# XiSHEN0220/RANSAC-Flow

Measured on AMD Instinct MI355X. Metric: aligned image-pairs/sec @480×640, 1/2/4/8 MI355X; max-abs flow Δ vs ref, higher is better.
Workload: dtype f32

## Files before the change

include/rfx_api.h:

```cpp
#ifndef RFX_API_H
#define RFX_API_H

#include <stddef.h>
#include <stdint.h>

#ifdef __cplusplus
extern "C" {
#endif

#define RFX_OK 0
#define RFX_E_ARG (-1)
#define RFX_E_LIMIT (-2)

#define RFX_ACT_NONE 0
#define RFX_ACT_RELU 1
#define RFX_ACT_SIGMOID 2

const char* rfx_version(void);

#define RFX_ABI_VERSION 17
int rfx_abi_version(void);

int rfx_group_begin(void);
int rfx_group_end(void* stream);
int rfx_group_abort(void);
int rfx_group_side_streams(int enable);
int rfx_group_stats(long long* groups, long long* launches);

int rfx_conv2d_f32(const float* in, const float* wT, const int32_t* ktab, const float* scale,
                   const float* shift, const float* residual, float* out, int N, int Cin, int Hin,
                   int Win, int Cout, int KH, int KW, int stride, int pad, int act, void* stream);

int rfx_conv2d_tile_variant(int N, int Cout, int Hout, int Wout);

int rfx_conv2d_kernel_id(int N, int Cin, int Cout, int KH, int KW, int stride, int pad, int Hout, int Wout);

int rfx_conv3x3_f32(const float* in, const float* wP, const float* scale, const float* shift, const float* residual,
                    float* out, int N, int Cin, int H, int W, int Cout, int act, int k_chunk, void* stream);
int rfx_conv3x3_kernel_id(int N, int Cin, int Cout, int H, int W, int k_chunk);
int rfx_conv3x3_s2_f32(const float* in, const float* wP, const float* scale, const float* shift, const float* residual,
                       float* out, int N, int Cin, int H, int W, int Cout, int act, void* stream);

int rfx_conv3x3_conv1x1_kernel_id(int N, int H, int W, int Cmid);
int rfx_conv3x3_conv1x1_f32(const float* in, const float* wP2, const float* scale2, const float* shift2, int act2,
                            const float* wQ3, const float* scale3, const float* shift3, const float* residual, int act3,
                            float* out, int N, int Cin, int H, int W, int Cmid, int Cexp, void* stream);

int rfx_maxpool2d_f32(const float* in, float* out, int NC, int Hin, int Win, int k, int stride,
                      int pad, void* stream);

int rfx_blurpool2d_f32(const float* in, float* out, int NC, int Hin, int Win, int stride, void* stream);

int rfx_maxblurpool2d_f32(const float* in, float* out, int NC, int Hin, int Win, int stride, void* stream);

int rfx_stem_conv3x3_maxblur_f32(const float* in, const float* wT, const float* scale, const float* shift, float* out,
                                 int N, int H, int W, int Cout, void* stream);

int rfx_stem_conv7x7_maxpool_f32(const float* in, const float* wT, const float* scale, const float* shift, float* out,
                                 int N, int H, int W, int Cout, void* stream);

int rfx_l2norm_nchw_f32(const float* in, float* out, int N, int C, int HW, long long out_batch_stride,
                        long long out_chan_stride, void* stream);
int rfx_l2norm_nchw_scatter_f32(const float* in, float* out, int N, int C, int HW, const long long* dst_off,
                                long long out_chan_stride, void* stream);

int rfx_flow_head_f32(const float* logits, float* flow, int N, int K, int rows, int cols, void* stream);

int rfx_resize_bilinear_f32(const float* in, float* out, int NC, int Hin, int Win, int Hout, int Wout,
                            int align_corners, void* stream);

int rfx_lanczos_pass_u8(const uint8_t* in, uint8_t* out, int N, int inH, int inW, int outH, int outW, int C,
                        const int32_t* bounds, const int32_t* weights, int ksize, int vertical, int row_offset,
                        void* stream);

int rfx_u8_to_f32_chw(const uint8_t* in, float* raw, float* norm, int N, int H, int W, const float* mean3_host,
                      const float* std3_host, void* stream);

int rfx_copy_cols_f32(const float* src, float* dst, long long rows, int w_src, int w_dst, void* stream);

int rfx_corr_neigh_f32(const float* x, const float* y, float* out, int N, int C, int H, int W, int K,
                       void* stream);
int rfx_corr_neigh_variant_f32(const float* x, const float* y, float* out, int N, int C, int H, int W, int K,
                               int variant, void* stream);

int rfx_corr_neigh_bidir_f32(const float* x, const float* y, float* out_xy, float* out_yx, int N, int C, int H, int W, int K,
                             void* stream);
int rfx_corr_timing(int enable);
int rfx_corr_timing_collect(float* us_out, int cap);

int rfx_warp_grid_f32(const float* Hm, float* grid, int B, int h, int w, void* stream);

int rfx_grid_sample_f32(const float* in, const float* grid, float* out, int N, int C, int Hi, int Wi,
                        int Ho, int Wo, int align_corners, void* stream);

int rfx_compose_flow_f32(const float* flowDown, const float* coarseGrid, float* flow12, float* inb,
                         float* flowUp, int N, int hd, int wd, int Hc, int Wc, int H, int W, int clamp, void* stream);

int rfx_flow_grad_clamp_f32(const float* flowCoarse, const float* grid, float* flowGrad, float* flow, int B, int H, int W,
                            int grid_batch, void* stream);

int rfx_merge_multi_h_f32(const float* flow, const float* match12, long long match12_stride, const float* cyc,
                          const float* inb, int n, long long HW, float th, int multiH, float* flowGlobal,
                          float* matchGlobal, uint8_t* binary, void* stream);

int rfx_match_score_f32(const float* match12, long long match12_stride, const float* cyc, const float* inb, int n,
                        long long HW, float* score, void* stream);

size_t rfx_remove_small_cc_ws_bytes(int N, int H, int W);
int rfx_remove_small_cc_f32(const float* in, float* out, int N, int H, int W, float match_th, int max_area, void* ws,
                            void* stream);

size_t rfx_remove_small_cc_ragged_ws_bytes(long long total_px);
int rfx_remove_small_cc_ragged_f32(const float* in, float* out, const long long* match_off, const int32_t* dims, int n_active,
                                   long long total_px, long long max_hw, float match_th, void* ws, void* stream);

size_t rfx_nearest_fill_ws_bytes(int N, int H, int W);
int rfx_nearest_fill_f32(const float* values, const unsigned char* explained, float* out, int32_t* index, int N, int H, int W, int C,
                         void* ws, void* stream);

size_t rfx_flow_points_ws_bytes(int N, int H, int W);
int rfx_flow_points_f32(const float* flow, const unsigned char* keep, const unsigned char* bg, int N, int H, int W, int k, int wA,
                        int hA, int wB, int hB, float* pts1, long long* pts2, long long* offsets, void* ws, void* stream);
// ... 131 lines not shown
```

ransac-flow_amd/csrc/pool.hip:

```cpp
#include "common.h"
#include "group.h"
#include <math.h>

static inline int grid_for(long long total, int block) {
    long long g = (total + block - 1) / block;
    const long long cap = 256LL * 32;
    return (int)(g < cap ? g : cap);
}

__global__ __launch_bounds__(256) void maxpool2d_kernel(const float* __restrict__ in, float* __restrict__ out,
                                                        long long total, int Hin, int Win, int Hout, int Wout,
                                                        int k, int stride, int pad) {
    for (long long idx = (long long)blockIdx.x * blockDim.x + threadIdx.x; idx < total;
         idx += (long long)gridDim.x * blockDim.x) {
        const int ow = (int)(idx % Wout);
        const long long r = idx / Wout;
        const int oh = (int)(r % Hout);
        const long long nc = r / Hout;
        const float* src = in + nc * Hin * Win;
        float m = -INFINITY;
        const int ih0 = oh * stride - pad, iw0 = ow * stride - pad;
        for (int i = 0; i < k; ++i) {
            const int ih = ih0 + i;
            if ((unsigned)ih >= (unsigned)Hin) continue;
            for (int j = 0; j < k; ++j) {
                const int iw = iw0 + j;
                if ((unsigned)iw >= (unsigned)Win) continue;
                const float v = src[(size_t)ih * Win + iw];
                m = (v > m || v != v) ? v : m;
            }
        }
        out[idx] = m;
    }
}

extern "C" int rfx_maxpool2d_f32(const float* in, float* out, int NC, int Hin, int Win, int k, int stride,
                                 int pad, void* stream) {
    if (!in || !out || NC <= 0 || Hin <= 0 || Win <= 0 || k <= 0 || stride <= 0 || pad < 0 || pad > k / 2)
        return RFX_E_ARG;
    const int Hout = (Hin + 2 * pad - k) / stride + 1, Wout = (Win + 2 * pad - k) / stride + 1;
    if (Hout <= 0 || Wout <= 0) return RFX_E_ARG;
    const long long total = (long long)NC * Hout * Wout;
    hipLaunchKernelGGL(maxpool2d_kernel, dim3(grid_for(total, 256)), dim3(256), 0, rfx_stream(stream), in, out,
                       total, Hin, Win, Hout, Wout, k, stride, pad);
    RFX_LAUNCH_CHECK();
    return RFX_OK;
}

__device__ __forceinline__ int reflect1(int i, int n) {
    return i < 0 ? -i : (i >= n ? 2 * n - 2 - i : i);
}

struct PlaneArgs { const float* in; float* out; long long total; int Hin, Win, Hout, Wout, stride; };
struct L2NormArgs { const float* in; float* out; long long NP; int C, HW; long long obs, ocs; };
struct FlowHeadArgs { const float* logits; float* flow; long long NP; int K, rows, cols; };
struct ResizeArgs { const float* in; float* out; long long total; int Hin, Win, Hout, Wout; float sh, sw; int align; };

__device__ __forceinline__ void blurpool2d_body(const PlaneArgs& a, const unsigned bx, const unsigned gx) {
    const long long total = a.total;
    const int Hin = a.Hin, Win = a.Win, Hout = a.Hout, Wout = a.Wout, stride = a.stride;
    const float w[3] = {0.25f, 0.5f, 0.25f};
    [&](const float* __restrict__ in, float* __restrict__ out) {
    for (long long idx = (long long)bx * blockDim.x + threadIdx.x; idx < total;
         idx += (long long)gx * blockDim.x) {
        const int ow = (int)(idx % Wout);
        const long long r = idx / Wout;
        const int oh = (int)(r % Hout);
        const long long nc = r / Hout;
        const float* src = in + nc * Hin * Win;
        float acc = 0.0f;
#pragma unroll
        for (int i = 0; i < 3; ++i) {
            const int ih = reflect1(oh * stride - 1 + i, Hin);
#pragma unroll
            for (int j = 0; j < 3; ++j) {
                const int iw = reflect1(ow * stride - 1 + j, Win);
                acc = fmaf(src[(size_t)ih * Win + iw], w[i] * w[j], acc);
            }
        }
        out[idx] = acc;
    }
    }(a.in, a.out);
}

using BlurPool = RfxFamily<PlaneArgs, blurpool2d_body, 256>;
__global__ __launch_bounds__(BlurPool::BLOCK) void blurpool2d_kernel(PlaneArgs a) { blurpool2d_body(a, blockIdx.x, gridDim.x); }

extern "C" int rfx_blurpool2d_f32(const float* in, float* out, int NC, int Hin, int Win, int stride, void* stream) {
    if (!in || !out || NC <= 0 || Hin < 2 || Win < 2 || stride <= 0) return RFX_E_ARG;
    const int Hout = (Hin + 2 - 3) / stride + 1, Wout = (Win + 2 - 3) / stride + 1;
    const long long total = (long long)NC * Hout * Wout;
    const PlaneArgs a = {in, out, total, Hin, Win, Hout, Wout, stride};
    return BlurPool::launch(blurpool2d_kernel, a, (unsigned)grid_for(total, BlurPool::BLOCK), rfx_stream(stream));
}

__global__ __launch_bounds__(256) void maxblurpool2d_kernel(const float* __restrict__ in, float* __restrict__ out,
                                                            long long total, int Hin, int Win, int Hout, int Wout,
                                                            int stride) {
    const float w[3] = {0.25f, 0.5f, 0.25f};
    const int Hm = Hin - 1, Wm = Win - 1;
    for (long long idx = (long long)blockIdx.x * blockDim.x + threadIdx.x; idx < total;
         idx += (long long)gridDim.x * blockDim.x) {
        const int ow = (int)(idx % Wout);
        const long long r = idx / Wout;
        const int oh = (int)(r % Hout);
        const long long nc = r / Hout;
        const float* src = in + nc * Hin * Win;
        float acc = 0.0f;
#pragma unroll
        for (int i = 0; i < 3; ++i) {
            const int my = reflect1(oh * stride - 1 + i, Hm);
#pragma unroll
            for (int j = 0; j < 3; ++j) {
                const int mx = reflect1(ow * stride - 1 + j, Wm);
                const float* q = src + (size_t)my * Win + mx;
                const float a = q[0], b = q[1], c = q[Win], d = q[Win + 1];
                float m = a;
                m = (b > m || b != b) ? b : m;
                m = (c > m || c != c) ? c : m;
                m = (d > m || d != d) ? d : m;
                acc = fmaf(m, w[i] * w[j], acc);
            }
        }
        out[idx] = acc;
    }
}

__device__ __forceinline__ float maxblur_one(const float* __restrict__ src, int oh, int ow, int Win, int Hm, int Wm) {
    const float w[3] = {0.25f, 0.5f, 0.25f};
    float acc = 0.0f;
#pragma unroll
    for (int i = 0; i < 3; ++i) {
        const int my = reflect1(oh * 2 - 1 + i, Hm);
#pragma unroll
        for (int j = 0; j < 3; ++j) {
            const int mx = reflect1(ow * 2 - 1 + j, Wm);
            const float* q = src + (size_t)my * Win + mx;
            const float a = q[0], b = q[1], c = q[Win], d = q[Win + 1];
            float m = a;
            m = (b > m || b != b) ? b : m;
            m = (c > m || c != c) ? c : m;
            m = (d > m || d != d) ? d : m;
            acc = fmaf(m, w[i] * w[j], acc);
        }
    }
    return acc;
}

__global__ __launch_bounds__(256) void maxblurpool2d_s2_block_kernel(const float* __restrict__ in,
                                                                     float* __restrict__ out, long long nblocks,
                                                                     int Hin, int Win, int Hout, int Wout) {
    const float w[3] = {0.25f, 0.5f, 0.25f};
    const int Hm = Hin - 1, Wm = Win - 1;
    const int BH = (Hout + 1) / 2, BW = (Wout + 1) / 2;
    for (long long idx = (long long)blockIdx.x * blockDim.x + threadIdx.x; idx < nblocks;
         idx += (long long)gridDim.x * blockDim.x) {
        const int bx = (int)(idx % BW);
        const long long r = idx / BW;
        const int by = (int)(r % BH);
        const long long nc = r / BH;
        const float* src = in + nc * Hin * Win;
        float* dst = out + nc * Hout * Wout;
        const bool interior = by >= 1 && 4 * by + 4 <= Hin - 1 && bx >= 1 && 4 * bx + 8 <= Win && 2 * by + 1 < Hout &&
                              2 * bx + 1 < Wout;
        if (!interior) {
#pragma unroll
            for (int dy = 0; dy < 2; ++dy)
#pragma unroll
                for (int dx = 0; dx < 2; ++dx) {
                    const int oh = 2 * by + dy, ow = 2 * bx + dx;
                    if (oh < Hout && ow < Wout) dst[(size_t)oh * Wout + ow] = maxblur_one(src, oh, ow, Win, Hm, Wm);
                }
            continue;
        }
// ... 329 lines not shown
```

ransac-flow_amd/csrc/preproc.hip:

```cpp
#include "common.h"

namespace {

constexpr int PRECISION_BITS = 32 - 8 - 2;

__device__ __forceinline__ uint8_t clip8(int v) {
    v >>= PRECISION_BITS;
    return (uint8_t)(v < 0 ? 0 : (v > 255 ? 255 : v));
}

template <int CT>
__global__ __launch_bounds__(256) void lanczos_pass_kernel(const uint8_t* __restrict__ in, uint8_t* __restrict__ out,
                                                           long long total, int inH, int inW, int oH, int oW, int Crt,
                                                           const int32_t* __restrict__ bounds,
                                                           const int32_t* __restrict__ kk, int ksize, int vertical,
                                                           int row_off) {
    for (long long idx = (long long)blockIdx.x * blockDim.x + threadIdx.x; idx < total;
         idx += (long long)gridDim.x * blockDim.x) {
        const int ox = (int)(idx % oW);
        const long long r = idx / oW;
        const int oy = (int)(r % oH);
        const long long n = r / oH;
        const int C = CT ? CT : Crt;
        const uint8_t* src = in + (size_t)n * inH * inW * C;
        const int o = vertical ? oy : ox;
        const int lo = bounds[2 * o], cnt = bounds[2 * o + 1];
        const int32_t* k = kk + (size_t)o * ksize;
        int acc[4] = {1 << (PRECISION_BITS - 1), 1 << (PRECISION_BITS - 1), 1 << (PRECISION_BITS - 1),
                      1 << (PRECISION_BITS - 1)};
        if (vertical) {
            for (int j = 0; j < cnt; ++j) {
                const uint8_t* p = src + ((size_t)(lo + j) * inW + ox) * C;
                const int w = k[j];
#pragma unroll
                for (int c = 0; c < 4; ++c) if (c < C) acc[c] += (int)p[c] * w;
            }
        } else {
            const uint8_t* row = src + (size_t)(oy + row_off) * inW * C;
            for (int j = 0; j < cnt; ++j) {
                const uint8_t* p = row + (size_t)(lo + j) * C;
                const int w = k[j];
#pragma unroll
                for (int c = 0; c < 4; ++c) if (c < C) acc[c] += (int)p[c] * w;
            }
        }
        uint8_t* dst = out + (size_t)idx * C;
#pragma unroll
        for (int c = 0; c < 4; ++c) if (c < C) dst[c] = clip8(acc[c]);
    }
}

__global__ __launch_bounds__(256) void u8_to_f32_kernel(const uint8_t* __restrict__ in, float* __restrict__ raw,
                                                        float* __restrict__ norm, long long total, int HW, float m0,
                                                        float m1, float m2, float s0, float s1, float s2) {
    const float mean[3] = {m0, m1, m2}, sd[3] = {s0, s1, s2};
    for (long long idx = (long long)blockIdx.x * blockDim.x + threadIdx.x; idx < total;
         idx += (long long)gridDim.x * blockDim.x) {
        const long long n = idx / HW;
        const int px = (int)(idx - n * HW);
        const uint8_t* p = in + (size_t)idx * 3;
#pragma unroll
        for (int c = 0; c < 3; ++c) {
            const float v = __fdiv_rn((float)p[c], 255.0f);
            const size_t o = ((size_t)n * 3 + c) * HW + px;
            if (raw) raw[o] = v;
            if (norm) norm[o] = __fdiv_rn(__fsub_rn(v, mean[c]), sd[c]);
        }
    }
}

inline int grid_for(long long total) {
    long long g = (total + 255) / 256;
    return (int)(g < 8192 ? g : 8192);
}

}

extern "C" int rfx_lanczos_pass_u8(const uint8_t* in, uint8_t* out, int N, int inH, int inW, int outH, int outW, int C,
                                   const int32_t* bounds, const int32_t* weights, int ksize, int vertical, int row_offset,
                                   void* stream) {
    if (!in || !out || !bounds || !weights) return RFX_E_ARG;
    if (N <= 0 || inH <= 0 || inW <= 0 || outH <= 0 || outW <= 0 || C <= 0 || C > 4 || ksize <= 0 || row_offset < 0)
        return RFX_E_ARG;
    if (vertical ? (outW != inW) : (outH + row_offset > inH)) return RFX_E_ARG;
    const long long total = (long long)N * outH * outW;
    if (C == 3)
        hipLaunchKernelGGL(lanczos_pass_kernel<3>, dim3(grid_for(total)), dim3(256), 0, rfx_stream(stream), in, out, total, inH,
                           inW, outH, outW, C, bounds, weights, ksize, vertical, row_offset);
    else
        hipLaunchKernelGGL(lanczos_pass_kernel<0>, dim3(grid_for(total)), dim3(256), 0, rfx_stream(stream), in, out, total, inH,
                           inW, outH, outW, C, bounds, weights, ksize, vertical, row_offset);
    RFX_LAUNCH_CHECK();
    return RFX_OK;
}

extern "C" int rfx_u8_to_f32_chw(const uint8_t* in, float* raw, float* norm, int N, int H, int W, const float* mean3_host,
                                 const float* std3_host, void* stream) {
    if (!in || (!raw && !norm) || N <= 0 || H <= 0 || W <= 0) return RFX_E_ARG;
    if (norm && (!mean3_host || !std3_host)) return RFX_E_ARG;
    const float one[3] = {1.f, 1.f, 1.f}, zero[3] = {0.f, 0.f, 0.f};
    const float* m = mean3_host ? mean3_host : zero;
    const float* s = std3_host ? std3_host : one;
    const long long total = (long long)N * H * W;
    hipLaunchKernelGGL(u8_to_f32_kernel, dim3(grid_for(total)), dim3(256), 0, rfx_stream(stream), in, raw, norm, total,
                       H * W, m[0], m[1], m[2], s[0], s[1], s[2]);
    RFX_LAUNCH_CHECK();
    return RFX_OK;
}
```

ransac-flow_amd/rfx/_lib.py:

```python
import ctypes
import os
from ctypes import c_int, c_int32, c_int64, c_uint64, c_float, c_double, c_void_p, c_size_t, c_longlong, c_char_p

_HERE = os.path.dirname(os.path.abspath(__file__))
LIB_PATH = os.environ.get("RFX_LIB") or os.path.normpath(os.path.join(_HERE, "..", "librfx.so"))

SIGNATURES = {
    "rfx_version": (c_char_p, []),
    "rfx_abi_version": (c_int, []),
    "rfx_group_begin": (c_int, []),
    "rfx_group_end": (c_int, [c_void_p]),
    "rfx_group_abort": (c_int, []),
    "rfx_group_side_streams": (c_int, [c_int]),
    "rfx_group_stats": (c_int, [c_void_p, c_void_p]),
    "rfx_conv2d_f32": (c_int, [c_void_p] * 7 + [c_int] * 10 + [c_void_p]),
    "rfx_conv2d_dilated_f32": (c_int, [c_void_p] * 7 + [c_int] * 11 + [c_void_p]),
    "rfx_conv1x1_split_f32": (c_int, [c_void_p] * 6 + [c_int] * 5 + [c_void_p]),
    "rfx_conv3x3_split_f32": (c_int, [c_void_p] * 6 + [c_int] * 6 + [c_void_p]),
    "rfx_conv3x3_split_s2_f32": (c_int, [c_void_p] * 6 + [c_int] * 6 + [c_void_p]),
    "rfx_conv1x1_split_strided_f32": (c_int, [c_void_p] * 6 + [c_int] * 7 + [c_void_p]),
    "rfx_conv1x1_split_tile_channels": (c_int, [c_int] * 4),
    "rfx_conv1x1_expand64_f32": (c_int, [c_void_p] * 6 + [c_int] * 6 + [c_void_p]),
    "rfx_conv1x1_expand64_dual_f32": (c_int, [c_void_p] * 9 + [c_int] * 5 + [c_void_p]),
    "rfx_adaptive_avgpool2d_f32": (c_int, [c_void_p, c_void_p] + [c_int] * 5 + [c_void_p]),
    "rfx_softmax_accum_f32": (c_int, [c_void_p, c_void_p, c_int, c_int, c_longlong, c_float, c_int, c_void_p]),
    "rfx_argmax_mask_f32": (c_int, [c_void_p, c_int, c_int, c_longlong, c_int, c_int, c_void_p, c_void_p, c_void_p]),
    "rfx_conv2d_tile_variant": (c_int, [c_int] * 4),
    "rfx_conv2d_kernel_id": (c_int, [c_int] * 9),
    "rfx_conv3x3_f32": (c_int, [c_void_p] * 6 + [c_int] * 7 + [c_void_p]),
    "rfx_conv3x3_kernel_id": (c_int, [c_int] * 6),
    "rfx_conv3x3_s2_f32": (c_int, [c_void_p] * 6 + [c_int] * 6 + [c_void_p]),
    "rfx_conv3x3_conv1x1_kernel_id": (c_int, [c_int] * 4),
    "rfx_conv3x3_conv1x1_f32": (c_int, [c_void_p] * 4 + [c_int] + [c_void_p] * 4 + [c_int, c_void_p] + [c_int] * 6 + [c_void_p]),
    "rfx_maxpool2d_f32": (c_int, [c_void_p, c_void_p] + [c_int] * 6 + [c_void_p]),
    "rfx_blurpool2d_f32": (c_int, [c_void_p, c_void_p] + [c_int] * 4 + [c_void_p]),
    "rfx_maxblurpool2d_f32": (c_int, [c_void_p, c_void_p] + [c_int] * 4 + [c_void_p]),
    "rfx_stem_conv3x3_maxblur_f32": (c_int, [c_void_p] * 5 + [c_int] * 4 + [c_void_p]),
    "rfx_stem_conv7x7_maxpool_f32": (c_int, [c_void_p] * 5 + [c_int] * 4 + [c_void_p]),
    "rfx_l2norm_nchw_f32": (c_int, [c_void_p, c_void_p, c_int, c_int, c_int, c_longlong, c_longlong, c_void_p]),
    "rfx_l2norm_nchw_scatter_f32": (c_int, [c_void_p, c_void_p, c_int, c_int, c_int, c_void_p, c_longlong, c_void_p]),
    "rfx_flow_head_f32": (c_int, [c_void_p, c_void_p] + [c_int] * 4 + [c_void_p]),
    "rfx_resize_bilinear_f32": (c_int, [c_void_p, c_void_p] + [c_int] * 6 + [c_void_p]),
    "rfx_lanczos_pass_u8": (c_int, [c_void_p, c_void_p] + [c_int] * 6 + [c_void_p, c_void_p] + [c_int] * 3 + [c_void_p]),
    "rfx_u8_to_f32_chw": (c_int, [c_void_p] * 3 + [c_int] * 3 + [c_void_p] * 3),
    "rfx_copy_cols_f32": (c_int, [c_void_p, c_void_p, c_longlong, c_int, c_int, c_void_p]),
    "rfx_corr_neigh_f32": (c_int, [c_void_p] * 3 + [c_int] * 5 + [c_void_p]),
    "rfx_corr_neigh_variant_f32": (c_int, [c_void_p] * 3 + [c_int] * 6 + [c_void_p]),
    "rfx_corr_neigh_bidir_f32": (c_int, [c_void_p] * 4 + [c_int] * 5 + [c_void_p]),
    "rfx_corr_timing": (c_int, [c_int]),
    "rfx_corr_timing_collect": (c_int, [c_void_p, c_int]),
    "rfx_warp_grid_f32": (c_int, [c_void_p, c_void_p] + [c_int] * 3 + [c_void_p]),
    "rfx_grid_sample_f32": (c_int, [c_void_p] * 3 + [c_int] * 7 + [c_void_p]),
    "rfx_compose_flow_f32": (c_int, [c_void_p] * 5 + [c_int] * 8 + [c_void_p]),
    "rfx_flow_grad_clamp_f32": (c_int, [c_void_p] * 4 + [c_int] * 4 + [c_void_p]),
    "rfx_merge_multi_h_f32": (c_int, [c_void_p, c_void_p, c_longlong, c_void_p, c_void_p, c_int, c_longlong, c_float, c_int,
                                      c_void_p, c_void_p, c_void_p, c_void_p]),
    "rfx_match_score_f32": (c_int, [c_void_p, c_longlong, c_void_p, c_void_p, c_int, c_longlong, c_void_p, c_void_p]),
    "rfx_remove_small_cc_ws_bytes": (c_size_t, [c_int] * 3),
    "rfx_remove_small_cc_f32": (c_int, [c_void_p, c_void_p, c_int, c_int, c_int, c_float, c_int, c_void_p, c_void_p]),
    "rfx_remove_small_cc_ragged_ws_bytes": (c_size_t, [c_longlong]),
    "rfx_remove_small_cc_ragged_f32": (c_int, [c_void_p] * 4 + [c_int, c_longlong, c_longlong, c_float, c_void_p, c_void_p]),
    "rfx_nearest_fill_ws_bytes": (c_size_t, [c_int] * 3),
    "rfx_nearest_fill_f32": (c_int, [c_void_p] * 4 + [c_int] * 4 + [c_void_p, c_void_p]),
    "rfx_flow_points_ws_bytes": (c_size_t, [c_int] * 3),
    "rfx_flow_points_f32": (c_int, [c_void_p] * 3 + [c_int] * 8 + [c_void_p] * 5),
    "rfx_sample_points_f32": (c_int, [c_void_p] * 4 + [c_int] * 5 + [c_void_p] * 4),
    "rfx_epe_ws_bytes": (c_size_t, [c_int] * 3),
    "rfx_epe_homography_f32": (c_int, [c_void_p] * 2 + [c_int] * 3 + [c_void_p] * 5),
    "rfx_epe_flow_f32": (c_int, [c_void_p] * 4 + [c_int] * 3 + [c_void_p] * 5),
    "rfx_mutual_nn_ws_bytes": (c_size_t, [c_int, c_int]),
    "rfx_mutual_nn_f32": (c_int, [c_void_p, c_int, c_int, c_void_p, c_int, c_int, c_int] + [c_void_p] * 5 + [c_int, c_void_p]),
    "rfx_mutual_nn_batched_f32": (c_int, [c_void_p, c_int, c_int, c_longlong, c_void_p, c_int, c_int, c_longlong, c_int]
                                  + [c_void_p] * 5 + [c_int, c_int, c_void_p]),
    "rfx_mutual_nn_ragged_f32": (c_int, [c_void_p, c_int, c_void_p, c_int, c_void_p, c_void_p, c_int, c_int, c_int, c_void_p,
                                         c_void_p, c_void_p, c_int, c_void_p, c_void_p, c_int, c_int, c_void_p]),
    "rfx_dlt4_homography": (c_int, [c_void_p, c_void_p, c_int, c_void_p, c_void_p]),
    "rfx_prediction_f32": (c_int, [c_void_p, c_void_p, c_int, c_void_p, c_int, c_void_p, c_void_p]),
    "rfx_score_hypotheses": (c_int, [c_void_p, c_void_p, c_int, c_void_p, c_int, c_float] + [c_void_p] * 5),
    "rfx_ransac_ws_bytes": (c_size_t, [c_int, c_int]),
    "rfx_ransac_h4": (c_int, [c_void_p, c_void_p, c_int, c_void_p, c_int, c_float] + [c_void_p] * 5),
    "rfx_ransac_batched_ws_bytes": (c_size_t, [c_int, c_int, c_int]),
    "rfx_ransac_h4_batched_stage": (c_int, [c_void_p, c_void_p, c_void_p, c_int, c_void_p, c_int, c_float] + [c_void_p] * 4
                                    + [c_int, c_int, c_void_p]),
    "rfx_ransac_degenerate_gather": (c_int, [c_void_p] * 4 + [c_int, c_void_p, c_int, c_int] + [c_void_p] * 5 + [c_int, c_void_p]),
    "rfx_ransac_patch_h_rows": (c_int, [c_void_p, c_int, c_int, c_int] + [c_void_p] * 4 + [c_int, c_void_p]),
    "rfx_dlt4_homography_flags": (c_int, [c_void_p, c_void_p, c_int, c_void_p, c_void_p, c_void_p]),
    "rfx_ransac_h4_batched": (c_int, [c_void_p, c_void_p, c_void_p, c_int, c_void_p, c_int, c_float] + [c_void_p] * 4
                              + [c_int, c_void_p]),
    "rfx_gather_matches_f32": (c_int, [c_void_p, c_void_p, c_void_p, c_int] + [c_void_p] * 6 + [c_int, c_void_p]),
    "rfx_gather_matches_ragged_f32": (c_int, [c_void_p, c_void_p, c_void_p, c_int] + [c_void_p] * 8 + [c_int, c_void_p]),
    "rfx_draw_samples_i64": (c_int, [c_void_p, c_void_p, c_int, c_int, c_uint64, c_uint64, c_void_p, c_void_p]),
    "rfx_filter_matches_f32": (c_int, [c_void_p, c_void_p, c_void_p, c_int, c_void_p, c_int, c_void_p, c_void_p] + [c_int] * 4
                               + [c_void_p] * 9),
    "rfx_keep_mask_f32": (c_int, [c_void_p] * 3 + [c_int] * 5 + [c_void_p, c_void_p]),
    "rfx_multih_accept_ws_bytes": (c_size_t, [c_int]),
    "rfx_multih_accept_f32": (c_int, [c_void_p] * 4 + [c_int] * 3 + [c_void_p] * 3 + [c_double, c_int] + [c_void_p] * 7
                              + [c_int, c_int, c_void_p, c_int, c_int, c_void_p, c_longlong] + [c_int] * 5 + [c_void_p]),
    "rfx_filter_matches_ragged_f32": (c_int, [c_void_p, c_void_p, c_void_p, c_int, c_void_p, c_int] + [c_void_p] * 15),
    "rfx_keep_mask_ragged_f32": (c_int, [c_void_p] * 5 + [c_int] * 3 + [c_void_p] * 3),
    "rfx_multih_accept_ragged_ws_bytes": (c_size_t, [c_int]),
    "rfx_multih_accept_ragged_f32": (c_int, [c_void_p] * 7 + [c_int, c_longlong] + [c_void_p] * 3 + [c_double, c_int]
                                     + [c_void_p] * 9 + [c_longlong] + [c_int] * 3 + [c_void_p]),
    "rfx_multih_accept_ragged_d2_f32": (c_int, [c_void_p] * 7 + [c_int, c_longlong] + [c_void_p] * 3 + [c_double, c_int]
                                        + [c_void_p] * 12 + [c_longlong] + [c_int] * 3 + [c_void_p]),
}

ABI_VERSION = 17

_lib = None


def load():
    global _lib
# ... 31 lines not shown
```

ransac-flow_amd/rfx/ops.py:

```python
import collections
import ctypes
import os
import threading

import torch

from . import _lib

ACT_NONE, ACT_RELU, ACT_SIGMOID = 0, 1, 2


def _stream(dev=None):
    return ctypes.c_void_p(torch.cuda.current_stream(dev).cuda_stream)


def _on_device(dev, fn, *args):
    if dev.index is not None and dev.index != torch.cuda.current_device():
        with torch.cuda.device(dev):
            return fn(*args, _stream(dev))
    return fn(*args, _stream())


def _call(name, dev, *args):
    _lib.check(_on_device(dev, getattr(_lib.load(), name), *args), name)
# ... 256 lines not shown
            if self.route == "fp32_3x3":
                self.wP = pack_wP(w).to(dev)
        self.w2d = w.reshape(self.Cout, self.Cin) if (self.KH == 1 and self.KW == 1) else None
        self._wq = None
        if bn is not None:
            invstd = 1.0 / torch.sqrt(bn["running_var"].detach().float().cpu() + eps)
            alpha = bn["weight"].detach().float().cpu() * invstd
            beta = bn["bias"].detach().float().cpu() - bn["running_mean"].detach().float().cpu() * alpha
            self.scale, self.shift = alpha.to(dev), beta.to(dev)
        elif bias is not None:
            self.scale, self.shift = torch.ones(self.Cout, dtype=torch.float32).to(dev), bias.detach().float().cpu().to(dev)
        else:
            self.scale = self.shift = None

    def quad_weights(self):
        if getattr(self, "_wq", None) is None:
            self._wq = pack_wQ(self.w2d).to(self._device)
        return self._wq

    def out_hw(self, H, W):
        eh, ew = (self.KH - 1) * self.dilation + 1, (self.KW - 1) * self.dilation + 1
        return (H + 2 * self.pad - eh) // self.stride + 1, (W + 2 * self.pad - ew) // self.stride + 1

    def __call__(self, x, residual=None, act=None, out=None):
        x = _dev(x, "conv input")
        N, C, H, W = x.shape
        if C != self.Cin:
            raise ValueError("conv expects %d input channels, got %d" % (self.Cin, C))
        Ho, Wo = self.out_hw(H, W)
        out = _out_or_new(out, (N, self.Cout, Ho, Wo), x, "conv")
        res = _dev(residual, "residual") if residual is not None else None
        if res is not None and res.shape != out.shape:
            raise ValueError("residual shape %s != output shape %s" % (tuple(res.shape), tuple(out.shape)))
        self._RUN[self.route](self, x, res, out, self.act if act is None else act)
        return out


    def _run_dilated(self, x, res, out, act):
        N, C, H, W = x.shape
        _call("rfx_conv2d_dilated_f32", _one_device(x, res, self.wT), _p(x), _p(self.wT), _p(self.ktab), _p(self.scale), _p(self.shift),
              _p(res), _p(out), N, C, H, W, self.Cout, self.KH, self.KW, self.stride, self.pad, self.dilation, act)

    def _run_split3x3(self, x, res, out, act):
        N, C, H, W = x.shape
        e0 = Profiler.begin(x)
        xin, Cp = x, C
        if C % 16:
            Cp = (C + 15) // 16 * 16
            xin = torch.zeros((N, Cp, H, W), dtype=torch.float32, device=x.device)
            xin[:, :C].copy_(x)
            launch_group.keep(xin)
        _call("rfx_conv3x3_split_f32" if self.stride == 1 else "rfx_conv3x3_split_s2_f32", _one_device(xin, res, self.wS), _p(xin),
              _p(self.wS), _p(self.scale), _p(self.shift), _p(res), _p(out), N, Cp, H, W, self.Cout, act)
        if e0 is not None:
            Ho, Wo = out.shape[2:]
            Profiler.record_conv(KID_SPLIT_3X3 | (2 if self.Cout > 64 else 1) | (4 if self.stride != 1 else 0),
                                 2.0 * N * Ho * Wo * self.Cout * self.Cin * 9, e0, (N, self.Cin, H, W, self.Cout, 3, self.stride),
                                 4.0 * (N * C * H * W + N * self.Cout * Ho * Wo * (2 if res is not None else 1)) + 54.0 * self.Cout * self.Cin)

    def _run_split1x1(self, x, res, out, act):
        N, C, H, W = x.shape
        e0 = Profiler.begin(x)
        if self.stride == 1:
            _call("rfx_conv1x1_split_f32", _one_device(x, res, self.wS), _p(x), _p(self.wS), _p(self.scale), _p(self.shift), _p(res), _p(out),
                  N, C, H * W, self.Cout, act)
        else:
            _call("rfx_conv1x1_split_strided_f32", _one_device(x, res, self.wS), _p(x), _p(self.wS), _p(self.scale), _p(self.shift), _p(res),
                  _p(out), N, C, H, W, self.Cout, self.stride, act)
        if e0 is not None:
            Ho, Wo = out.shape[2:]
            Profiler.record_conv(KID_SPLIT_1X1 | (2 if self.Cout > 64 else 1) | (4 if self.stride != 1 else 0),
                                 2.0 * N * Ho * Wo * self.Cout * self.Cin, e0, (N, self.Cin, H, W, self.Cout, 1, self.stride),
                                 4.0 * (N * C * Ho * Wo + N * self.Cout * Ho * Wo * (2 if res is not None else 1)) + 6.0 * self.Cout * self.Cin)

    def _run_fp32_3x3(self, x, res, out, act):
        N, C, H, W = x.shape
        Ho, Wo = out.shape[2:]
        lib = _lib.load()
        kid0 = (lib.rfx_conv3x3_kernel_id(N, self.Cin, self.Cout, Ho, Wo, self.k_chunk) if self.stride == 1 else
                lib.rfx_conv2d_kernel_id(N, self.Cin, self.Cout, self.KH, self.KW, self.stride, self.pad, Ho, Wo))
        if not kid0 & (KID_DIRECT_3X3 | KID_DIRECT_3X3_S2):
            return self._run_gemm(x, res, out, act)
        e0 = Profiler.begin(x)
        if kid0 & KID_DIRECT_3X3:
            _call("rfx_conv3x3_f32", _one_device(x, res, self.wP), _p(x), _p(self.wP), _p(self.scale), _p(self.shift),
                  _p(res), _p(out), N, C, H, W, self.Cout, act, self.k_chunk)
        else:
            _call("rfx_conv3x3_s2_f32", _one_device(x, res, self.wP), _p(x), _p(self.wP), _p(self.scale), _p(self.shift),
                  _p(res), _p(out), N, C, H, W, self.Cout, act)
        if e0 is not None:
            self._record_fp32(kid0, e0, x, res, out)

    def _run_gemm(self, x, res, out, act):
        N, C, H, W = x.shape
        e0 = Profiler.begin(x)
        _call("rfx_conv2d_f32", _one_device(x, res, self.wT), _p(x), _p(self.wT), _p(self.ktab), _p(self.scale),
              _p(self.shift), _p(res), _p(out), N, C, H, W, self.Cout, self.KH, self.KW, self.stride, self.pad, act)
        if e0 is not None:
            self._record_fp32(0, e0, x, res, out)

    def _record_fp32(self, kid0, e0, x, res, out):
        N, C, H, W = x.shape
        Ho, Wo = out.shape[2:]
        kid = kid0 if (kid0 & KID_DIRECT_3X3) else _lib.load().rfx_conv2d_kernel_id(N, self.Cin, self.Cout, self.KH, self.KW, self.stride, self.pad, Ho, Wo)
        flops = 2.0 * N * Ho * Wo * self.Cout * self.Cin * self.KH * self.KW
        nbytes = 4.0 * (N * C * H * W + N * self.Cout * Ho * Wo * (2 if res is not None else 1)
                        + self.Cout * self.Cin * self.KH * self.KW)
        Profiler.record_conv(kid, flops, e0, (N, self.Cin, H, W, self.Cout, self.KH, self.stride), nbytes)

    _RUN = {"dilated": _run_dilated, "split3x3": _run_split3x3, "split3x3_s2": _run_split3x3, "split1x1": _run_split1x1,
            "fp32_3x3": _run_fp32_3x3, "gemm": _run_gemm}


ConvGeometry = collections.namedtuple("ConvGeometry", "Cout Cin KH KW stride pad act scale")


def bottleneck_tail_shape(plan2, plan3):
    return (plan2.KH == 3 and plan2.KW == 3 and plan2.stride == 1 and plan2.pad == 1 and plan2.Cin % 8 == 0
            and plan2.Cout in (64, 128) and plan2.act in (ACT_NONE, ACT_RELU) and plan3.KH == 1 and plan3.KW == 1
            and plan3.stride == 1 and plan3.pad == 0 and plan3.Cin == plan2.Cout and plan3.Cout % 128 == 0
            and plan3.act in (ACT_NONE, ACT_RELU) and plan3.scale is not None)


def bottleneck_tail_eligible(plan2, plan3):
    return (bottleneck_tail_shape(plan2, plan3) and os.environ.get("RFX_FUSE_BOTTLENECK", "1") != "0"
            and getattr(plan2, "wS", None) is None and getattr(plan3, "wS", None) is None)


def bottleneck_tail(x, plan2, plan3, residual=None):
    x = _dev(x, "bottleneck input")
    N, C, H, W = x.shape
    if C != plan2.Cin:
        raise ValueError("conv expects %d input channels, got %d" % (plan2.Cin, C))
    res = _dev(residual, "residual") if residual is not None else None
    out = torch.empty((N, plan3.Cout, H, W), dtype=torch.float32, device=x.device)
    if res is not None and res.shape != out.shape:
        raise ValueError("residual shape %s != output shape %s" % (tuple(res.shape), tuple(out.shape)))
    e0 = Profiler.begin(x)
    _call("rfx_conv3x3_conv1x1_f32", _one_device(x, res, plan2.wP, plan3.scale), _p(x), _p(plan2.wP), _p(plan2.scale),
          _p(plan2.shift), plan2.act, _p(plan3.quad_weights()), _p(plan3.scale), _p(plan3.shift), _p(res), plan3.act,
          _p(out), N, C, H, W, plan2.Cout, plan3.Cout)
    if e0 is not None:
        Profiler.record_conv(_lib.load().rfx_conv3x3_conv1x1_kernel_id(N, H, W, plan2.Cout),
                             2.0 * N * H * W * (plan2.Cout * plan2.Cin * 9 + plan3.Cout * plan3.Cin), e0, (N, C, H, W, plan3.Cout, 3, 1),
                             4.0 * N * H * W * (C + plan3.Cout * (2 if res is not None else 1)))
    return out


_EXPAND64 = None


def expand64_enabled():
    global _EXPAND64
    if _EXPAND64 is None:
        _EXPAND64 = os.environ.get("RFX_EXPAND64", "1") != "0"
    return _EXPAND64


def expand64_eligible(plan):
    return (plan.KH == 1 and plan.KW == 1 and plan.stride == 1 and plan.pad == 0 and getattr(plan, "dilation", 1) == 1
            and plan.Cin == 64 and plan.Cout % 256 == 0 and plan.Cout <= 256 and plan.scale is not None
            and plan.act in (ACT_NONE, ACT_RELU))


EXPAND64_MIN_PIXELS = {"plain": 300000, "dual": 100000}


def expand64_form(plan3, plan_ds=None, pixels=None):
    def ok(p):
        return expand64_eligible(p) and getattr(p, "route", "gemm") == "gemm"
    if not expand64_enabled() or not ok(plan3) or plan3.act != ACT_RELU:
        return None
    if plan_ds is not None:
        form = "dual" if (ok(plan_ds) and plan_ds.act == ACT_NONE and plan_ds.Cout == plan3.Cout) else None
    else:
        form = "plain"
    if form is not None and pixels is not None and pixels < EXPAND64_MIN_PIXELS[form]:
        return None
    return form


def conv1x1_expand64(x, plan, residual=None, shortcut=None):
    if residual is not None and shortcut is not None:
        raise ValueError("conv1x1_expand64: a residual or a shortcut, not both")
    x = _dev(x, "conv input")
    N, C, H, W = x.shape
    plan_s = shortcut[1] if shortcut is not None else None
    form = expand64_form(plan, plan_s, N * H * W)
    if getattr(launch_group._tls, "active", None) is not None:
        form = None
    if form is None:
        return plan(x, residual=plan_s(shortcut[0]) if shortcut is not None else residual)
    if C != plan.Cin:
        raise ValueError("conv expects %d input channels, got %d" % (plan.Cin, C))
    out = torch.empty((N, plan.Cout, H, W), dtype=torch.float32, device=x.device)
    e0 = Profiler.begin(x)
    if form == "dual":
        xs = _dev(shortcut[0], "shortcut input")
        if xs.shape != x.shape:
            raise ValueError("shortcut input shape %s != conv input shape %s" % (tuple(xs.shape), tuple(x.shape)))
        _call("rfx_conv1x1_expand64_dual_f32", _one_device(x, xs, plan.wT, plan_s.wT), _p(x), _p(plan.wT), _p(plan.scale), _p(plan.shift),
              _p(xs), _p(plan_s.wT), _p(plan_s.scale), _p(plan_s.shift), _p(out), N, C, H * W, plan.Cout, 1)
    else:
        res = _dev(residual, "residual") if residual is not None else None
        if res is not None and res.shape != out.shape:
            raise ValueError("residual shape %s != output shape %s" % (tuple(res.shape), tuple(out.shape)))
        _call("rfx_conv1x1_expand64_f32", _one_device(x, res, plan.wT), _p(x), _p(plan.wT), _p(plan.scale), _p(plan.shift), _p(res), _p(out),
              N, C, H * W, plan.Cout, 1, plan.act)
    if e0 is not None:
        gemms = 2 if form == "dual" else 1
        planes = plan.Cout * (2 if (form == "plain" and residual is not None) else 1)
        Profiler.record_conv(_lib.load().rfx_conv2d_kernel_id(N, plan.Cin, plan.Cout, 1, 1, 1, 0, H, W),
                             gemms * 2.0 * N * H * W * plan.Cout * plan.Cin, e0, (N, plan.Cin, H, W, plan.Cout, 1, 1),
                             4.0 * (N * H * W * (gemms * C + planes) + gemms * plan.Cout * plan.Cin))
    return out


def maxpool2d(x, k, stride, pad=0):
    x = _dev(x, "maxpool input")
    N, C, H, W = x.shape
    Ho, Wo = (H + 2 * pad - k) // stride + 1, (W + 2 * pad - k) // stride + 1
    out = torch.empty((N, C, Ho, Wo), dtype=torch.float32, device=x.device)
    _call("rfx_maxpool2d_f32", x.device, _p(x), _p(out), N * C, H, W, k, stride, pad)
    return out


def blurpool2d(x, stride=2):
    x = _dev(x, "blurpool input")
    N, C, H, W = x.shape
# ... 1134 lines not shown
```

Before: 164.5.

## Add specialized thin conv3x3, stride-2 blurpool quad kernel, and tiled Lanczos resize kernels

Adds a dedicated 3x3 conv kernel for single-output-channel layers. It stages double-buffered input patches and weights in shared memory so one output map no longer goes through the general direct kernel. A stride-2 blurpool kernel computes four outputs per thread with vectorized row loads and stores. New vertical and horizontal Lanczos preprocessing kernels pack bytes and tile pixels and weights in shared memory. All three are on by default behind env switches, with fallbacks when group recording is active or limits are exceeded. The thin kernel hardcodes a weight stride of 128 (Mpad) that may not match every plan layout.

```diff
diff --git a/include/rfx_api.h b/include/rfx_api.h
--- a/include/rfx_api.h
+++ b/include/rfx_api.h
@@ -38,6 +38,8 @@
 int rfx_conv3x3_f32(const float* in, const float* wP, const float* scale, const float* shift, const float* residual,
                     float* out, int N, int Cin, int H, int W, int Cout, int act, int k_chunk, void* stream);
 int rfx_conv3x3_kernel_id(int N, int Cin, int Cout, int H, int W, int k_chunk);
+int rfx_conv3x3_thin_f32(const float* in, const float* wT, const float* scale, const float* shift, float* out, int N, int Cin,
+                         int H, int W, int Cout, int act, void* stream);
 int rfx_conv3x3_s2_f32(const float* in, const float* wP, const float* scale, const float* shift, const float* residual,
                        float* out, int N, int Cin, int H, int W, int Cout, int act, void* stream);
 
diff --git a/ransac-flow_amd/csrc/conv3x3t.hip b/ransac-flow_amd/csrc/conv3x3t.hip
--- /dev/null
+++ b/ransac-flow_amd/csrc/conv3x3t.hip
@@ -0,0 +1,87 @@
+#include "common.h"
+
+namespace {
+
+struct C3TArgs {
+    const float* in;
+    const float* wT;
+    const float* scale;
+    const float* shift;
+    float* out;
+    int Cin, H, W, Mpad, act;
+};
+
+constexpr int TP = 16, PP = TP + 2, CB = 8;
+constexpr int PATCH = CB * PP * PP;
+constexpr int NLD = (PATCH + 255) / 256;
+constexpr int C3T_MAX_CIN = 256;
+
+__global__ __launch_bounds__(256, 4) void conv3x3_thin_kernel(C3TArgs a) {
+    __shared__ __attribute__((aligned(16))) float s_w[C3T_MAX_CIN * 9];
+    __shared__ float s_x[2][PATCH];
+    const int t = threadIdx.x, tx = t & (TP - 1), ty = t >> 4;
+    const int x0 = blockIdx.x * TP, y0 = blockIdx.y * TP;
+    const int H = a.H, W = a.W, HW = H * W, K = a.Cin * 9;
+    const float* __restrict__ img = a.in + (size_t)blockIdx.z * a.Cin * HW;
+
+    int off[NLD];
+#pragma unroll
+    for (int i = 0; i < NLD; ++i) {
+        const int e = t + 256 * i, c = e / (PP * PP), r = e - c * (PP * PP), py = r / PP, px = r - py * PP;
+        const int iy = y0 + py - 1, ix = x0 + px - 1;
+        off[i] = (e < PATCH && iy >= 0 && iy < H && ix >= 0 && ix < W) ? c * HW + iy * W + ix : -1;
+    }
+    float v[NLD];
+    auto fetch = [&](int c0) {
+        const float* __restrict__ p = img + (size_t)c0 * HW;
+#pragma unroll
+        for (int i = 0; i < NLD; ++i) v[i] = off[i] >= 0 ? p[off[i]] : 0.0f;
+    };
+    auto stash = [&](int buf) {
+#pragma unroll
+        for (int i = 0; i < NLD; ++i)
+            if (t + 256 * i < PATCH) s_x[buf][t + 256 * i] = v[i];
+    };
+    fetch(0);
+    for (int k = t; k < K; k += 256) s_w[k] = a.wT[(size_t)k * a.Mpad];
+    stash(0);
+    __syncthreads();
+
+    float acc = 0.0f;
+    const int nst = a.Cin / CB;
+    for (int s = 0; s < nst; ++s) {
+        if (s + 1 < nst) fetch((s + 1) * CB);
+        const float* xs = &s_x[s & 1][ty * PP + tx];
+        const float* ws = &s_w[s * (CB * 9)];
+#pragma unroll 2
+        for (int c = 0; c < CB; ++c)
+#pragma unroll
+            for (int kh = 0; kh < 3; ++kh)
+#pragma unroll
+                for (int kw = 0; kw < 3; ++kw) acc = fmaf(ws[c * 9 + kh * 3 + kw], xs[c * (PP * PP) + kh * PP + kw], acc);
+        if (s + 1 < nst) stash((s + 1) & 1);
+        __syncthreads();
+    }
+
+    const int oy = y0 + ty, ox = x0 + tx;
+    if (oy >= H || ox >= W) return;
+    float r = fmaf(acc, a.scale ? a.scale[0] : 1.0f, a.shift ? a.shift[0] : 0.0f);
+    if (a.act == RFX_ACT_RELU) r = r > 0.0f ? r : 0.0f;
+    else if (a.act == RFX_ACT_SIGMOID) r = 1.0f / (1.0f + expf(-r));
+    a.out[(size_t)blockIdx.z * HW + (size_t)oy * W + ox] = r;
+}
+
+}
+
+extern "C" int rfx_conv3x3_thin_f32(const float* in, const float* wT, const float* scale, const float* shift, float* out, int N,
+                                    int Cin, int H, int W, int Cout, int act, void* stream) {
+    if (!in || !wT || !out || N <= 0 || H <= 0 || W <= 0) return RFX_E_ARG;
+    if (Cout != 1 || Cin < CB || Cin % CB != 0) return RFX_E_ARG;
+    if (act != RFX_ACT_NONE && act != RFX_ACT_RELU && act != RFX_ACT_SIGMOID) return RFX_E_ARG;
+    if (Cin > C3T_MAX_CIN || N > 65535 || rfx_cdiv(H, TP) > 65535 || (long long)Cin * H * W > 0x7fffffffLL) return RFX_E_LIMIT;
+    const C3TArgs a = {in, wT, scale, shift, out, Cin, H, W, 128, act};
+    hipLaunchKernelGGL(conv3x3_thin_kernel, dim3((unsigned)rfx_cdiv(W, TP), (unsigned)rfx_cdiv(H, TP), (unsigned)N), dim3(256), 0,
+                       rfx_stream(stream), a);
+    RFX_LAUNCH_CHECK();
+    return RFX_OK;
+}
diff --git a/ransac-flow_amd/csrc/pool.hip b/ransac-flow_amd/csrc/pool.hip
--- a/ransac-flow_amd/csrc/pool.hip
+++ b/ransac-flow_amd/csrc/pool.hip
@@ -86,10 +86,80 @@
 using BlurPool = RfxFamily<PlaneArgs, blurpool2d_body, 256>;
 __global__ __launch_bounds__(BlurPool::BLOCK) void blurpool2d_kernel(PlaneArgs a) { blurpool2d_body(a, blockIdx.x, gridDim.x); }
 
+__device__ __forceinline__ float blur_one_s2(const float* __restrict__ src, int oh, int ow, int Hin, int Win) {
+    const float w[3] = {0.25f, 0.5f, 0.25f};
+    float acc = 0.0f;
+#pragma unroll
+    for (int i = 0; i < 3; ++i) {
+        const int ih = reflect1(oh * 2 - 1 + i, Hin);
+#pragma unroll
+        for (int j = 0; j < 3; ++j) {
+            const int iw = reflect1(ow * 2 - 1 + j, Win);
+            acc = fmaf(src[(size_t)ih * Win + iw], w[i] * w[j], acc);
+        }
+    }
+    return acc;
+}
+
+__global__ __launch_bounds__(256) void blurpool2d_s2_quad_kernel(const float* __restrict__ in, float* __restrict__ out, int NC,
+                                                                 int Hin, int Win, int Hout, int Wout, int Q, int vec, int vst) {
+    const float w[3] = {0.25f, 0.5f, 0.25f};
+    const unsigned t = blockIdx.x * 256u + threadIdx.x;
+    const unsigned oh = t / (unsigned)Q;
+    if (oh >= (unsigned)Hout) return;
+    const int q = (int)(t - oh * (unsigned)Q), ow0 = 4 * q;
+    const bool interior = vec && oh >= 1 && 2 * (int)oh + 1 <= Hin - 1 && q >= 1 && 8 * q + 7 <= Win - 1 && ow0 + 3 < Wout;
+    for (int nc = blockIdx.y; nc < NC; nc += gridDim.y) {
+        const float* src = in + (size_t)nc * Hin * Win;
+        float* dst = out + (size_t)nc * Hout * Wout + (size_t)oh * Wout + ow0;
+        if (!interior) {
+#pragma unroll
+            for (int d = 0; d < 4; ++d)
+                if (ow0 + d < Wout) dst[d] = blur_one_s2(src, (int)oh, ow0 + d, Hin, Win);
+            continue;
+        }
+        const float* p = src + (size_t)(2 * oh - 1) * Win + 8 * q;
+        float v[3][9];
+#pragma unroll
+        for (int i = 0; i < 3; ++i) {
+            const float* r = p + (size_t)i * Win;
+            const f32x4 a4 = *reinterpret_cast<const f32x4*>(r), b4 = *reinterpret_cast<const f32x4*>(r + 4);
+            v[i][0] = r[-1];
+            v[i][1] = a4[0]; v[i][2] = a4[1]; v[i][3] = a4[2]; v[i][4] = a4[3];
+            v[i][5] = b4[0]; v[i][6] = b4[1]; v[i][7] = b4[2]; v[i][8] = b4[3];
+        }
+        f32x4 o;
+#pragma unroll
+        for (int d = 0; d < 4; ++d) {
+            float acc = 0.0f;
+#pragma unroll
+            for (int i = 0; i < 3; ++i)
+#pragma unroll
+                for (int j = 0; j < 3; ++j) acc = fmaf(v[i][2 * d + j], w[i] * w[j], acc);
+            o[d] = acc;
+        }
+        if (vst) {
+            *reinterpret_cast<f32x4*>(dst) = o;
+        } else {
+            dst[0] = o[0]; dst[1] = o[1]; dst[2] = o[2]; dst[3] = o[3];
+        }
+    }
+}
+
 extern "C" int rfx_blurpool2d_f32(const float* in, float* out, int NC, int Hin, int Win, int stride, void* stream) {
     if (!in || !out || NC <= 0 || Hin < 2 || Win < 2 || stride <= 0) return RFX_E_ARG;
     const int Hout = (Hin + 2 - 3) / stride + 1, Wout = (Win + 2 - 3) / stride + 1;
     const long long total = (long long)NC * Hout * Wout;
+    static const bool fast = !(getenv("RFX_BLURPOOL_FAST") && atoi(getenv("RFX_BLURPOOL_FAST")) == 0);
+    const int Q = (Wout + 3) / 4;
+    if (fast && stride == 2 && !rfx_group_recording() && (long long)Hout * Q <= 0x7fffff00LL) {
+        const int vec = Win % 4 == 0 && (reinterpret_cast<uintptr_t>(in) & 15) == 0;
+        const int vst = Wout % 4 == 0 && (reinterpret_cast<uintptr_t>(out) & 15) == 0;
+        hipLaunchKernelGGL(blurpool2d_s2_quad_kernel, dim3((unsigned)rfx_cdiv((long long)Hout * Q, 256), (unsigned)(NC < 32768 ? NC : 32768)),
+                           dim3(256), 0, rfx_stream(stream), in, out, NC, Hin, Win, Hout, Wout, Q, vec, vst);
+        RFX_LAUNCH_CHECK();
+        return RFX_OK;
+    }
     const PlaneArgs a = {in, out, total, Hin, Win, Hout, Wout, stride};
     return BlurPool::launch(blurpool2d_kernel, a, (unsigned)grid_for(total, BlurPool::BLOCK), rfx_stream(stream));
 }
diff --git a/ransac-flow_amd/csrc/preproc.hip b/ransac-flow_amd/csrc/preproc.hip
--- a/ransac-flow_amd/csrc/preproc.hip
+++ b/ransac-flow_amd/csrc/preproc.hip
@@ -50,6 +50,148 @@
     }
 }
 
+struct LzAcc {
+    unsigned lo;
+    int hi;
+    __device__ __forceinline__ void tap(unsigned px, unsigned wlo, int whi) {
+        lo += __umul24(px, wlo);
+        hi += __mul24((int)px, whi);
+    }
+    __device__ __forceinline__ unsigned out() const {
+        return clip8((int)(((unsigned)hi << 16) + lo + (1u << (PRECISION_BITS - 1))));
+    }
+};
+
+__device__ __forceinline__ unsigned pack4(unsigned b0, unsigned b1, unsigned b2, unsigned b3) {
+    asm volatile("" : "+v"(b0), "+v"(b1), "+v"(b2), "+v"(b3));
+    return b0 | (b1 << 8) | (b2 << 16) | (b3 << 24);
+}
+
+__device__ __forceinline__ unsigned ld32(const uint8_t* p) { unsigned v; __builtin_memcpy(&v, p, 4); return v; }
+__device__ __forceinline__ void st32(uint8_t* p, unsigned v) { __builtin_memcpy(p, &v, 4); }
+
+__global__ __launch_bounds__(256) void lanczos_v3_kernel(const uint8_t* __restrict__ in, uint8_t* __restrict__ out, int inH, int RB,
+                                                         int oH, const int32_t* __restrict__ bounds,
+                                                         const int32_t* __restrict__ kk, int ksize) {
+    const int oy = __builtin_amdgcn_readfirstlane(blockIdx.y * 4 + threadIdx.y);
+    const int xb = (blockIdx.x * 64 + threadIdx.x) * 4;
+    if (oy >= oH || xb >= RB) return;
+    const int lo = bounds[2 * oy], cnt = bounds[2 * oy + 1];
+    const int32_t* k = kk + (size_t)oy * ksize;
+    const uint8_t* src = in + ((size_t)blockIdx.z * inH + lo) * RB + xb;
+    uint8_t* dst = out + ((size_t)blockIdx.z * oH + oy) * RB + xb;
+    LzAcc a[4] = {{0u, 0}, {0u, 0}, {0u, 0}, {0u, 0}};
+    if (xb + 4 <= RB) {
+        for (int j = 0; j < cnt; ++j) {
+            const unsigned v = ld32(src + (size_t)j * RB);
+            const int w = k[j];
+            const unsigned wlo = (unsigned)w & 0xffffu;
+            const int whi = w >> 16;
+            a[0].tap(v & 255u, wlo, whi);
+            a[1].tap((v >> 8) & 255u, wlo, whi);
+            a[2].tap((v >> 16) & 255u, wlo, whi);
+            a[3].tap(v >> 24, wlo, whi);
+        }
+        st32(dst, pack4(a[0].out(), a[1].out(), a[2].out(), a[3].out()));
+    } else {
+        const int nb = RB - xb;
+        for (int j = 0; j < cnt; ++j) {
+            const int w = k[j];
+            const unsigned wlo = (unsigned)w & 0xffffu;
+            const int whi = w >> 16;
+#pragma unroll
+            for (int b = 0; b < 3; ++b) if (b < nb) a[b].tap(src[(size_t)j * RB + b], wlo, whi);
+        }
+#pragma unroll
+        for (int b = 0; b < 3; ++b) if (b < nb) dst[b] = (uint8_t)a[b].out();
+    }
+}
+
+constexpr int LZH_S = 64, LZH_R = 16, LZH_SPAN = 192, LZH_KS = 32;
+
+__global__ __launch_bounds__(256) void lanczos_h3_kernel(const uint8_t* __restrict__ in, uint8_t* __restrict__ out, int inH, int inW,
+                                                         int oH, int oW, const int32_t* __restrict__ bounds,
+                                                         const int32_t* __restrict__ kk, int ksize, int row_off) {
+    __shared__ unsigned s_px[LZH_R][LZH_SPAN];
+    __shared__ unsigned s_wlo[LZH_S * LZH_KS];
+    __shared__ int s_whi[LZH_S * LZH_KS];
+    const int t = threadIdx.x, col = t & 63, rg = t >> 6;
+    const int x0 = blockIdx.x * LZH_S, y0 = blockIdx.y * LZH_R;
+    const int ncol = min(LZH_S, oW - x0), nrow = min(LZH_R, oH - y0);
+    const uint8_t* src = in + ((size_t)blockIdx.z * inH + y0 + row_off) * inW * 3;
+    uint8_t* dst = out + (((size_t)blockIdx.z * oH + y0) * oW + x0) * 3;
+    const int lo = col < ncol ? bounds[2 * (x0 + col)] : 0x7fffffff, cnt = col < ncol ? bounds[2 * (x0 + col) + 1] : 0;
+    int pmin = lo, pend = col < ncol ? lo + cnt : (int)0x80000000;
+#pragma unroll
+    for (int m = 32; m >= 1; m >>= 1) {
+        pmin = min(pmin, __shfl_xor(pmin, m));
+        pend = max(pend, __shfl_xor(pend, m));
+    }
+    const int span = pend - pmin;
+    if (span > LZH_SPAN || span < 0 || ksize > LZH_KS || pmin < 0) {
+        if (col < ncol) {
+            const int32_t* k = kk + (size_t)(x0 + col) * ksize;
+            for (int r = rg; r < nrow; r += 4) {
+                const uint8_t* row = src + (size_t)r * inW * 3;
+                LzAcc a[3] = {{0u, 0}, {0u, 0}, {0u, 0}};
+                for (int j = 0; j < cnt; ++j) {
+                    const int w = k[j];
+                    const uint8_t* p = row + (size_t)(lo + j) * 3;
+#pragma unroll
+                    for (int ch = 0; ch < 3; ++ch) a[ch].tap(p[ch], (unsigned)w & 0xffffu, w >> 16);
+                }
+                uint8_t* d = dst + ((size_t)r * oW + col) * 3;
+#pragma unroll
+                for (int ch = 0; ch < 3; ++ch) d[ch] = (uint8_t)a[ch].out();
+            }
+        }
+        return;
+    }
+    {
+        const int r = t >> 4;
+        if (r < nrow) {
+            const uint8_t* row = src + (size_t)r * inW * 3 + (size_t)pmin * 3;
+#pragma unroll 4
+            for (int i = t & 15; i < span; i += 16)
+                s_px[r][i] = (unsigned)row[3 * i] | ((unsigned)row[3 * i + 1] << 8) | ((unsigned)row[3 * i + 2] << 16);
+        }
+    }
+#pragma unroll 2
+    for (int i = t; i < ncol * ksize; i += 256) {
+        const int w = kk[(size_t)x0 * ksize + i];
+        s_wlo[i] = (unsigned)w & 0xffffu;
+        s_whi[i] = w >> 16;
+    }
+    __syncthreads();
+    if (col >= ncol) return;
+    const int l = lo - pmin, c = min(cnt, ksize);
+    LzAcc a[LZH_R / 4][3];
+#pragma unroll
+    for (int u = 0; u < LZH_R / 4; ++u)
+#pragma unroll
+        for (int ch = 0; ch < 3; ++ch) a[u][ch] = {0u, 0};
+    for (int j = 0; j < c; ++j) {
+        const unsigned wlo = s_wlo[col * ksize + j];
+        const int whi = s_whi[col * ksize + j];
+#pragma unroll
+        for (int u = 0; u < LZH_R / 4; ++u) {
+            const unsigned v = s_px[rg + 4 * u][l + j];
+            a[u][0].tap(v & 255u, wlo, whi);
+            a[u][1].tap((v >> 8) & 255u, wlo, whi);
+            a[u][2].tap(v >> 16, wlo, whi);
+        }
+    }
+#pragma unroll
+    for (int u = 0; u < LZH_R / 4; ++u) {
+        const int r = rg + 4 * u;
+        if (r < nrow) {
+            uint8_t* d = dst + ((size_t)r * oW + col) * 3;
+#pragma unroll
+            for (int ch = 0; ch < 3; ++ch) d[ch] = (uint8_t)a[u][ch].out();
+        }
+    }
+}
+
 __global__ __launch_bounds__(256) void u8_to_f32_kernel(const uint8_t* __restrict__ in, float* __restrict__ raw,
                                                         float* __restrict__ norm, long long total, int HW, float m0,
                                                         float m1, float m2, float s0, float s1, float s2) {
@@ -84,6 +226,17 @@
         return RFX_E_ARG;
     if (vertical ? (outW != inW) : (outH + row_offset > inH)) return RFX_E_ARG;
     const long long total = (long long)N * outH * outW;
+    static const bool fast = !(getenv("RFX_LANCZOS_FAST") && atoi(getenv("RFX_LANCZOS_FAST")) == 0);
+    if (fast && C == 3 && N <= 65535 && outH <= 262140 && inW <= (1 << 28) && outW <= (1 << 28)) {
+        if (vertical)
+            hipLaunchKernelGGL(lanczos_v3_kernel, dim3((unsigned)rfx_cdiv(rfx_cdiv(inW * 3LL, 4), 64), (unsigned)rfx_cdiv(outH, 4), (unsigned)N),
+                               dim3(64, 4), 0, rfx_stream(stream), in, out, inH, inW * 3, outH, bounds, weights, ksize);
+        else
+            hipLaunchKernelGGL(lanczos_h3_kernel, dim3((unsigned)rfx_cdiv(outW, LZH_S), (unsigned)rfx_cdiv(outH, LZH_R), (unsigned)N),
+                               dim3(256), 0, rfx_stream(stream), in, out, inH, inW, outH, outW, bounds, weights, ksize, row_offset);
+        RFX_LAUNCH_CHECK();
+        return RFX_OK;
+    }
     if (C == 3)
         hipLaunchKernelGGL(lanczos_pass_kernel<3>, dim3(grid_for(total)), dim3(256), 0, rfx_stream(stream), in, out, total, inH,
                            inW, outH, outW, C, bounds, weights, ksize, vertical, row_offset);
diff --git a/ransac-flow_amd/rfx/_lib.py b/ransac-flow_amd/rfx/_lib.py
--- a/ransac-flow_amd/rfx/_lib.py
+++ b/ransac-flow_amd/rfx/_lib.py
@@ -29,6 +29,7 @@
     "rfx_conv2d_kernel_id": (c_int, [c_int] * 9),
     "rfx_conv3x3_f32": (c_int, [c_void_p] * 6 + [c_int] * 7 + [c_void_p]),
     "rfx_conv3x3_kernel_id": (c_int, [c_int] * 6),
+    "rfx_conv3x3_thin_f32": (c_int, [c_void_p] * 5 + [c_int] * 6 + [c_void_p]),
     "rfx_conv3x3_s2_f32": (c_int, [c_void_p] * 6 + [c_int] * 6 + [c_void_p]),
     "rfx_conv3x3_conv1x1_kernel_id": (c_int, [c_int] * 4),
     "rfx_conv3x3_conv1x1_f32": (c_int, [c_void_p] * 4 + [c_int] + [c_void_p] * 4 + [c_int, c_void_p] + [c_int] * 6 + [c_void_p]),
diff --git a/ransac-flow_amd/rfx/ops.py b/ransac-flow_amd/rfx/ops.py
--- a/ransac-flow_amd/rfx/ops.py
+++ b/ransac-flow_amd/rfx/ops.py
@@ -362,7 +362,10 @@
         if not kid0 & (KID_DIRECT_3X3 | KID_DIRECT_3X3_S2):
             return self._run_gemm(x, res, out, act)
         e0 = Profiler.begin(x)
-        if kid0 & KID_DIRECT_3X3:
+        if kid0 & KID_DIRECT_3X3 and res is None and conv_thin_eligible(self, kid0, N, H * W) and not launch_group.recording():
+            _call("rfx_conv3x3_thin_f32", _one_device(x, self.wT), _p(x), _p(self.wT), _p(self.scale), _p(self.shift), _p(out),
+                  N, C, H, W, self.Cout, act)
+        elif kid0 & KID_DIRECT_3X3:
             _call("rfx_conv3x3_f32", _one_device(x, res, self.wP), _p(x), _p(self.wP), _p(self.scale), _p(self.shift),
                   _p(res), _p(out), N, C, H, W, self.Cout, act, self.k_chunk)
         else:
@@ -425,6 +428,24 @@
                              2.0 * N * H * W * (plan2.Cout * plan2.Cin * 9 + plan3.Cout * plan3.Cin), e0, (N, C, H, W, plan3.Cout, 3, 1),
                              4.0 * N * H * W * (C + plan3.Cout * (2 if res is not None else 1)))
     return out
+
+
+_CONV_THIN = None
+KID_CHUNKED = 16384
+CONV_THIN_MIN_IMAGES = 1
+
+
+def conv_thin_enabled():
+    global _CONV_THIN
+    if _CONV_THIN is None:
+        _CONV_THIN = os.environ.get("RFX_CONV_THIN", "1") != "0"
+    return _CONV_THIN
+
+
+def conv_thin_eligible(plan, kid0, N, pixels):
+    return (conv_thin_enabled() and plan.Cout == 1 and plan.KH == 3 and plan.KW == 3 and plan.stride == 1 and plan.pad == 1
+            and plan.Cin % 8 == 0 and 8 <= plan.Cin <= 256 and plan.k_chunk == 0 and not kid0 & KID_CHUNKED
+            and CONV_THIN_MIN_IMAGES <= N <= 65535 and plan.Cin * pixels < 2 ** 31 and pixels < 2 ** 20)
 
 
 _EXPAND64 = None
```

After: 165.9, median of 6. Within noise of the previous version (+0.9%).
